# young-how/DQN-based-UAV-3D_path_planer

Hardware: NVIDIA H100
Metric: env steps/sec (+ DQN updates/sec), 500x500x100 city (higher is better)
Workload: dtype f64 env state / f32 obs+learner

## Files before the change

### dqn-based-uav-3d_path_planer_b200/csrc/tc_forward.cu

```cuda
#include "tc_forward.cuh"
#include "env_block.cuh"

#include <stdlib.h>
#include <string.h>

#include "tma.cuh"
#include "wgmma.cuh"

namespace uavrl {

static inline int rup(int x, int m) { return (x + m - 1) / m * m; }

size_t tc_smem_bytes(const TcNet &tc) { return (size_t)2 * tc.a_bytes + (size_t)tc.img_bytes + (size_t)tc.max_rows * tc.acc_ld * 4; }

int tc_build(const uavrl_learner_config &c, const NetDev &net, TcNet &tc, std::vector<int32_t> &hi_map, std::vector<int32_t> &lo_map,
             std::vector<int32_t> &hi2_map, std::vector<int32_t> &lo2_map)
{
    memset(&tc, 0, sizeof(tc));
    tc.n_layers = net.n_layers; tc.in_dim = net.in_dim; tc.n_actions = net.n_actions; tc.dueling = net.dueling;
    if (net.in_dim % 4 != 0) return -1;
    int off = 0, maxK = 0, k_pad = rup(net.in_dim, 8);
    for (int l = 0; l < net.n_layers; ++l) {
        const LayerDev &L = net.L[l];
        TcLayer &T = tc.L[l];
// ... 61 lines not shown
                if (l > 0) {
                    hi2_map[pi] = elem(T.N_pad, T.t_hi_off, k, o);
                    lo2_map[pi] = elem(T.N_pad, T.t_lo_off, k, o);
                }
            }
            hi_map[vrow ? (size_t)L.b2_off + (o - out_main) : (size_t)L.b_off + o] = tc.bias_base / 4 + T.bias_off + o;
        }
    }
    (void)c;
    return 0;
}


#define TC_TRACE(slot) do { if (a.trace && blockIdx.x == 0 && threadIdx.x == 0) a.trace[slot] = clock64(); } while (0)

template <bool FUSE_ENV, bool ACT, bool DUELING, bool FIXED>
__global__ void __launch_bounds__(kTcThreads, 1) tc_forward_kernel_t(TcNet tc, TcArgs a, EnvFuse ef)
{
    TC_TRACE(0);
    extern __shared__ __align__(1024) unsigned char smem[];
    unsigned char *Ahi = smem, *Alo = smem + tc.a_bytes, *W = smem + 2 * tc.a_bytes;
    float *acc = reinterpret_cast<float *>(W + tc.img_bytes);
    __shared__ uint64_t wbar, wbar2;
    __shared__ const float *rows[kTcTile];
    __shared__ float s_rew[kTcTile], s_done[kTcTile];

    const int tid = threadIdx.x, warp = tid >> 5, lane = tid & 31, quad = warp & 3, half = warp >> 2;
    constexpr int kCtl = kTcThreads - 32;
    const bool early_w = (a.pdl & kPdlEarlyWeights) != 0;
    const uint32_t w_split = tc.n_layers > 1 ? (uint32_t)tc.L[1].hi_off : (uint32_t)tc.img_bytes;
    auto stage_image = [&]() {
        fence_proxy_async();
// ... 71 lines not shown
            waited = true;
            if (tid == kCtl && !early_w) stage_image();
        }
        if (!wready) {
            __syncthreads();
            mbar_wait(&wbar, 0);
            wready = true;
        }
        TC_TRACE(3);
        fence_proxy_async();
        __syncthreads();
        TC_TRACE(4);

        for (int l = 0; l < tc.n_layers; ++l) {
            const TcLayer T = tc.L[l];
            mma_3xtf32<kMmaFwd, FIXED>(acc, tc.acc_ld, Ahi, Alo, W + T.hi_off, W + T.lo_off, mma_sbo(T.K_pad), T.N_pad, T.K_pad / 8, R);
            TC_TRACE(5 + 3 * l);
            if (!w2ready) { if (w_split < (uint32_t)tc.img_bytes) mbar_wait(&wbar2, 0); w2ready = true; }
            TC_TRACE(6 + 3 * l);
            const float *bias = bias_all + T.bias_off;
            const int row = quad * 32 + lane;
            const bool live = quad * 32 < R;
            if (l + 1 < tc.n_layers) {
                const uint32_t sbon = mma_sbo(T.N_pad);
                const EpiSlice e(R, kTcThreads);
                for (int c = e.c0; c < T.N_pad; c += e.step) {
                    const float4 v = e.ld(acc, tc.acc_ld, c);
                    float4 h, lo4;
                    const float x0 = fmaxf(v.x + bias[c + 0], 0.f), x1 = fmaxf(v.y + bias[c + 1], 0.f);
                    const float x2 = fmaxf(v.z + bias[c + 2], 0.f), x3 = fmaxf(v.w + bias[c + 3], 0.f);
                    tf32_split(x0, h.x, lo4.x); tf32_split(x1, h.y, lo4.y); tf32_split(x2, h.z, lo4.z); tf32_split(x3, h.w, lo4.w);
// ... 57 lines not shown
                }
                __syncthreads();
            }
        }
        if (FUSE_ENV) {
            __shared__ EnvSmem<32> env_sm;
            for (int sb = 0; sb < R; sb += 32)
                env_block<true, 32, kTcThreads, false, 8>(ef.d, env_sm, base + sb, tid, UAVRL_ACT_DISCRETE27, a.actions, ef.obs_next,
                                                       ef.reward, ef.done, nullptr, nullptr, nullptr);
            __syncthreads();
        }
    }
    TC_TRACE(20);
}

bool tc_fixed_chains(const TcNet &tc, bool train)
{
    for (int l = 0; l < tc.n_layers; ++l) {
        const TcLayer &T = tc.L[l];
        if (!mma_fixed_product(kMmaFwd, T.N_pad, T.K_pad / 8)) return false;
        if (train && l > 0 && !mma_fixed_product(kMmaDx, T.K_pad, T.N_pad / 8)) return false;
    }
    return true;
}

typedef void (*ForwardKernel)(TcNet, TcArgs, EnvFuse);
template <bool F, bool A, bool D>
static ForwardKernel pick_fwd_x(bool fixed) { return fixed ? tc_forward_kernel_t<F, A, D, true> : tc_forward_kernel_t<F, A, D, false>; }
template <bool F, bool A>
static ForwardKernel pick_fwd_d(bool dueling, bool fixed) { return dueling ? pick_fwd_x<F, A, true>(fixed) : pick_fwd_x<F, A, false>(fixed); }
static ForwardKernel pick_forward_kernel(bool fuse_env, bool act, bool dueling, bool fixed)
{
    if (fuse_env) return pick_fwd_d<true, true>(dueling, fixed);
    return act ? pick_fwd_d<false, true>(dueling, fixed) : pick_fwd_d<false, false>(dueling, fixed);
}

int launch_tc_forward(uavrl_learner *l, const TcArgs &a_in, cudaStream_t st, const EnvFuse *fuse)
{
    TcArgs a = a_in;
    const int n_sm = num_sms();
    a.rows_per_tile = (a.n >= 128 * n_sm && l->tc.max_rows == 128) ? 128 : (a.n >= 64 * n_sm) ? 64 : 32;
    a.n_tiles = (a.n + a.rows_per_tile - 1) / a.rows_per_tile;
    const int grid = a.n_tiles < n_sm ? a.n_tiles : n_sm;
    static const bool trace_on = getenv("UAVRL_TC_TRACE") != nullptr;
    long long *tr = nullptr;
    if (trace_on) { UAVRL_CUDA(cudaMalloc((void **)&tr, 32 * sizeof(long long))); UAVRL_CUDA(cudaMemset(tr, 0, 32 * sizeof(long long))); a.trace = tr; }
    const int prev = (l->pdl_chain && g_pdl.load()) ? l->pdl_prev : kPdlNone;
    a.pdl = 0;
    if (prev != kPdlNone) {
        a.pdl = kPdlOn;
        if (a.mode == kTcAct) {
            if (prev == kPdlAdam) a.pdl |= kPdlEarlyRows;
            else if (prev == kPdlEnv) a.pdl |= kPdlEarlyWeights;
        } else if (prev == kPdlEnv || prev == kPdlTd) {
            a.pdl |= kPdlEarlyWeights;
        }
    }
    EnvFuse ef;
    memset(&ef, 0, sizeof(ef));
    if (fuse) {
        ef = *fuse;
        UAVRL_CUDA(launch_kernel(pick_forward_kernel(true, a.mode == kTcAct, l->tc.dueling != 0, tc_fixed_chains(l->tc, false)), dim3(grid), dim3(kTcThreads), tc_smem_bytes(l->tc), st, a.pdl != 0, l->tc, a, ef));
        l->pdl_prev = l->pdl_chain ? kPdlEnv : kPdlNone;
    } else {
        UAVRL_CUDA(launch_kernel(pick_forward_kernel(false, a.mode == kTcAct, l->tc.dueling != 0, tc_fixed_chains(l->tc, false)), dim3(grid), dim3(kTcThreads), tc_smem_bytes(l->tc), st, a.pdl != 0, l->tc, a, ef));
        l->pdl_prev = l->pdl_chain ? (a.mode == kTcAct ? kPdlAct : kPdlTd) : kPdlNone;
    }
    UAVRL_LAUNCHED();
    if (trace_on) {
        long long h[32];
        UAVRL_CUDA(cudaStreamSynchronize(st));
        UAVRL_CUDA(cudaMemcpy(h, tr, sizeof(h), cudaMemcpyDeviceToHost));
        cudaFree(tr);
        fprintf(stderr, "[tc_trace] mode=%d n=%d R=%d grid=%d cycles since start:", a.mode, a.n, a.rows_per_tile, grid);
        for (int i = 1; i < 32; ++i) if (h[i]) fprintf(stderr, " [%d]=%lld", i, h[i] - h[0]);
        fprintf(stderr, "\n");
    }
    return 0;
}

// ... 5 lines not shown
    if (tc_smem_bytes(l->tc) > 227 * 1024) return 0;
    const size_t P = (size_t)l->net.P;
    const size_t img = (size_t)l->tc.train_img_bytes;
    UAVRL_CUDA(cudaMalloc((void **)&l->tc_img_local, img));
    UAVRL_CUDA(cudaMalloc((void **)&l->tc_img_target, img));
    UAVRL_CUDA(cudaMemset(l->tc_img_local, 0, img));
    UAVRL_CUDA(cudaMemset(l->tc_img_target, 0, img));
    int32_t **maps[] = { &l->tc_hi_map, &l->tc_lo_map, &l->tc_hi2_map, &l->tc_lo2_map };
    std::vector<int32_t> *src[] = { &hi, &lo, &hi2, &lo2 };
    for (int i = 0; i < 4; ++i) {
        UAVRL_CUDA(cudaMalloc((void **)maps[i], P * 4));
        UAVRL_CUDA(cudaMemcpy(*maps[i], src[i]->data(), P * 4, cudaMemcpyHostToDevice));
    }
    UAVRL_CUDA(cudaMalloc((void **)&l->y_buf, (size_t)l->cfg.batch_size * 4));
    UAVRL_CUDA(cudaMalloc((void **)&l->astar_buf, (size_t)l->cfg.batch_size * 4));
    const bool fixed = tc_fixed_chains(l->tc, false);
    for (int ac = 0; ac < 2; ++ac)
        for (int du = 0; du < 2; ++du)
            UAVRL_CUDA(cudaFuncSetAttribute(pick_forward_kernel(false, ac != 0, du != 0, fixed), cudaFuncAttributeMaxDynamicSharedMemorySize,
                                            (int)tc_smem_bytes(l->tc)));
    {
        l->fuse_ok = true;
        for (int du = 0; du < 2; ++du) {
            cudaFuncAttributes fa;
            UAVRL_CUDA(cudaFuncGetAttributes(&fa, pick_forward_kernel(true, true, du != 0, fixed)));
            if (fa.sharedSizeBytes + tc_smem_bytes(l->tc) > (size_t)227 * 1024) l->fuse_ok = false;
        }
        if (l->fuse_ok)
            for (int du = 0; du < 2; ++du)
                UAVRL_CUDA(cudaFuncSetAttribute(pick_forward_kernel(true, true, du != 0, fixed), cudaFuncAttributeMaxDynamicSharedMemorySize,
                                                (int)tc_smem_bytes(l->tc)));
    }
    l->y_cap = l->cfg.batch_size;
    l->tc_ok = true;
    return tc_train_init(l);
}

}
```

### dqn-based-uav-3d_path_planer_b200/csrc/tc_forward.cuh

```cuda
#pragma once
#include <vector>

#include "env.cuh"
#include "learner.cuh"

namespace uavrl {

constexpr int kTcThreads = 256;
constexpr int kTcTile = 128;

enum TcMode { kTcAct = 0, kTcArgmax = 1, kTcTdMax = 2, kTcTdGather = 3 };

struct TcArgs {
    const unsigned char *img;
    BatchSrc src;
    const float *obs;
    int32_t n, n_tiles, mode, use_next, rows_per_tile;
    float eps; int32_t is_train;
    const float *u_tape; const int32_t *rand_tape;
    uint64_t key, call;
    int32_t *actions;
    float *q_out;
    float *y_out;
    float gamma;
    int32_t pdl;
    long long *trace;
};

int tc_build(const uavrl_learner_config &c, const NetDev &net, TcNet &tc, std::vector<int32_t> &hi_map, std::vector<int32_t> &lo_map,
             std::vector<int32_t> &hi2_map, std::vector<int32_t> &lo2_map);
int tc_train_init(uavrl_learner *l);
int launch_tc_train(uavrl_learner *l, const BatchSrc &src, int B, int global_batch, const float *y, int *n_grad_parts,
                    int *n_loss_parts, cudaStream_t st, cudaEvent_t after_chain = nullptr, const AdamArgs *adam = nullptr,
                    float *loss_out = nullptr, bool *adam_done = nullptr, bool fused_td = false);
bool tc_train_can_fuse_td(const uavrl_learner *l, int B);
size_t tc_smem_bytes(const TcNet &tc);
bool tc_fixed_chains(const TcNet &tc, bool train);
struct EnvFuse { EnvDev d; float *obs_next; float *reward; uint8_t *done; };
int launch_tc_forward(uavrl_learner *l, const TcArgs &a, cudaStream_t st, const EnvFuse *fuse = nullptr);
int tc_init(uavrl_learner *l);

}
```

### dqn-based-uav-3d_path_planer_b200/csrc/tc_train.cu

```cuda
#include <string.h>
#include <stdlib.h>

#include <atomic>

#include "tc_forward.cuh"
#include "tma.cuh"
#include "wgmma.cuh"

namespace uavrl {

constexpr int kDwChunk = 128;

struct TcTrainArgs {
    const unsigned char *img;
    BatchSrc src;
    int32_t B, R, n_tiles;
    const float *y;
    float inv_global_b;
    float *act_buf, *dz_buf;
    float *loss_partials;
    int32_t loss_kind;
    int32_t fused_td, algo;
    float gamma;
    const unsigned char *img_target;
// ... 78 lines not shown
    for (int u = 0; u < 4; ++u) {
        const int i = threadIdx.x + u * kTcThreads;
        if (i < total) {
            const int r = i & (R - 1), j = i >> lgR;
            float4 h, l;
            tf32_split(v[u].x, h.x, l.x); tf32_split(v[u].y, h.y, l.y); tf32_split(v[u].z, h.z, l.z); tf32_split(v[u].w, h.w, l.w);
            const uint32_t off = mma_off(r, 4 * j, sbo);
            *reinterpret_cast<float4 *>(Ahi + off) = h;
            *reinterpret_cast<float4 *>(Alo + off) = l;
        }
    }
}

__device__ __forceinline__ uint32_t nl_split(const TcNet &tc) { return tc.n_layers > 1 ? (uint32_t)tc.L[1].hi_off : (uint32_t)tc.img_bytes; }

template <int NPRE, bool DUELING, bool FIXED>
__global__ void __launch_bounds__(kTcThreads, 1) tc_train_kernel(TcNet tc, TcTrainArgs a)
{
    TR_TRACE(0);
    extern __shared__ __align__(1024) unsigned char smem[];
    const int R = a.R;
    const uint32_t a_bytes = (uint32_t)(R / 8) * mma_sbo(tc.max_k);
    unsigned char *Ahi = smem, *Alo = smem + a_bytes, *W = smem + 2 * a_bytes;
    float *acc = reinterpret_cast<float *>(W + tc.train_img_bytes);
    __shared__ uint64_t wbar, wbar2, wbar3;
    __shared__ const float *rows[kTcTile];
    __shared__ const float *rows2[kTcTile];
    __shared__ int s_act[kTcTile], s_astar[kTcTile];
    __shared__ uint8_t s_fresh[kTcTile];
    __shared__ float s_y[kTcTile], s_rew[kTcTile], s_done[kTcTile];
    __shared__ float s_loss;

    const int tid = threadIdx.x, warp = tid >> 5, lane = tid & 31, quad = warp & 3, half = warp >> 2;
    constexpr int kCtl = kTcThreads - 32;
    if (tid == 0) s_loss = 0.f;
    constexpr bool fused = NPRE > 0;
    constexpr int n_pre = NPRE;
    uint32_t wphase = 0;
    if (tid == kCtl) {
        mbar_init(&wbar, 1); mbar_init(&wbar2, 1); mbar_init(&wbar3, 1); fence_barrier_init();
        fence_proxy_async();
        if (!fused) bulk_g2s_chunked(W, a.img, (uint32_t)tc.train_img_bytes, &wbar);
        else {
            bulk_g2s_chunked(W, (n_pre == 2) ? a.img : a.img_target, (uint32_t)tc.img_bytes, &wbar);
            if (tc.train_img_bytes > tc.img_bytes)
// ... 41 lines not shown
        for (int pass = 0; pass < n_pre; ++pass) {
            if (pass > 0 && tid == kTcThreads - 32) {
                fence_proxy_async();
                bulk_g2s_chunked(W, a.img_target, (uint32_t)tc.img_bytes, &wbar);
            }
            if (pass == 0 && early_rows) a0_store(vnext, R, tc.L[0].K_pad, Ahi, Alo);
            else build_a0(rows2, R, tc.in_dim, tc.L[0].K_pad, Ahi, Alo);
            if (pass == 0) { park_meta(); TR_TRACE(3); }
            mbar_wait(&wbar, wphase); wphase ^= 1;
            fence_proxy_async();
            __syncthreads();
            if (pass == 0) TR_TRACE(4);
            const bool td_pass = (pass == n_pre - 1);
            for (int l = 0; l < nl; ++l) {
                const TcLayer T = tc.L[l];
                mma_3xtf32<kMmaFwd, FIXED>(acc, tc.acc_ld, Ahi, Alo, W + T.hi_off, W + T.lo_off, mma_sbo(T.K_pad), T.N_pad, T.K_pad / 8, R);
                const float *bias = bias_all + T.bias_off;
                if (l + 1 < nl) {
                    const uint32_t sbon = mma_sbo(T.N_pad);
                    for (int c = e.c0; c < T.N_pad; c += e.step) {
                        const float4 v = e.ld(acc, tc.acc_ld, c);
                        float4 x, h, lo4;
                        x.x = fmaxf(v.x + bias[c + 0], 0.f); x.y = fmaxf(v.y + bias[c + 1], 0.f);
                        x.z = fmaxf(v.z + bias[c + 2], 0.f); x.w = fmaxf(v.w + bias[c + 3], 0.f);
                        tf32_split(x.x, h.x, lo4.x); tf32_split(x.y, h.y, lo4.y); tf32_split(x.z, h.z, lo4.z); tf32_split(x.w, h.w, lo4.w);
                        const uint32_t off = mma_off(e.row, c, sbon);
                        *reinterpret_cast<float4 *>(Ahi + off) = h;
                        *reinterpret_cast<float4 *>(Alo + off) = lo4;
                    }
                } else if (half == 0 && live) {
                    float q[32];
// ... 40 lines not shown
        if (!waited) { pdl_wait(); pdl_trigger(); waited = true; }
        if (n_pre == 0) park_meta();
        if (!fused && tid < R) s_y[tid] = (base + tid < a.B) ? a.y[base + tid] : 0.f;
        if (fused) { mbar_wait(&wbar, wphase); wphase ^= 1; }
        else if (!wready) { mbar_wait(&wbar, 0); wready = true; }
        fence_proxy_async();
        __syncthreads();
        TR_TRACE(10);
        const int gb = base + row;
        const bool mine = live && gb < a.B;
        const int egb = base + e.row;
        const bool emine = egb < a.B;

        for (int l = 0; l < nl; ++l) {
            const TcLayer T = tc.L[l];
            mma_3xtf32<kMmaFwd, FIXED>(acc, tc.acc_ld, Ahi, Alo, W + T.hi_off, W + T.lo_off, mma_sbo(T.K_pad), T.N_pad, T.K_pad / 8, R);
            if (fused && l == 0 && w_split < (uint32_t)tc.img_bytes) mbar_wait(&wbar2, 0);
            if (l < 4) TR_TRACE(27 + l);
            const float *bias = bias_all + T.bias_off;
            if (l + 1 < nl) {
                const uint32_t sbon = mma_sbo(T.N_pad);
                float *act_row = a.act_buf + (size_t)egb * tc.act_stride + tc.L[l + 1].act_off;
                uint32_t mk = 0u;
                for (int c = e.c0, sh = 0; c < T.N_pad; c += e.step, sh += 4) {
                    const float4 v = e.ld(acc, tc.acc_ld, c);
                    float4 x, h, lo4;
                    x.x = fmaxf(v.x + bias[c + 0], 0.f); x.y = fmaxf(v.y + bias[c + 1], 0.f);
                    x.z = fmaxf(v.z + bias[c + 2], 0.f); x.w = fmaxf(v.w + bias[c + 3], 0.f);
                    tf32_split(x.x, h.x, lo4.x); tf32_split(x.y, h.y, lo4.y); tf32_split(x.z, h.z, lo4.z); tf32_split(x.w, h.w, lo4.w);
                    const uint32_t off = mma_off(e.row, c, sbon);
                    *reinterpret_cast<float4 *>(Ahi + off) = h;
// ... 32 lines not shown
                        if (a.src.abs_err) a.src.abs_err[gb] = fabsf(diff);
                        if (a.loss_kind == 0) {
                            lterm = wb * (diff * diff);
                            gq = (2.f * diff * wb) * a.inv_global_b;
                        } else {
                            const float ad = fabsf(diff);
                            lterm = wb * (ad < 1.f ? 0.5f * (diff * diff) : ad - 0.5f);
                            gq = (fminf(fmaxf(diff, -1.f), 1.f) * wb) * a.inv_global_b;
                        }
                    }
#pragma unroll
                    for (int off = 16; off > 0; off >>= 1) lterm += __shfl_xor_sync(0xffffffffu, lterm, off);
                    TR_TRACE(23);
                    if (lane == 0) atomicAdd(&s_loss, lterm);
                    TR_TRACE(24);
                    float g[32];
                    const float inv = 1.f / (float)nA;
#pragma unroll
                    for (int j = 0; j < 32; ++j) {
                        float gj;
                        if (DUELING) gj = (j < nA) ? gq * ((j == act ? 1.f : 0.f) - inv) : (j == nA ? gq : 0.f);
                        else gj = (j == act) ? gq : 0.f;
                        g[j] = gj;
                    }
                    TR_TRACE(25);
                    float *dz_row = a.dz_buf + (size_t)gb * tc.dz_stride + T.dz_off;
#pragma unroll
                    for (int j = 0; j < 8; ++j) {
                        float4 x = make_float4(g[4 * j], g[4 * j + 1], g[4 * j + 2], g[4 * j + 3]), h, lo4;
                        tf32_split(x.x, h.x, lo4.x); tf32_split(x.y, h.y, lo4.y); tf32_split(x.z, h.z, lo4.z); tf32_split(x.w, h.w, lo4.w);
                        const uint32_t off = mma_off(row, 4 * j, sbon);
                        *reinterpret_cast<float4 *>(Ahi + off) = h;
                        *reinterpret_cast<float4 *>(Alo + off) = lo4;
                        if (mine) *reinterpret_cast<float4 *>(dz_row + 4 * j) = x;
                    }
                    TR_TRACE(26);
                }
            }
            fence_proxy_async();
            __syncthreads();
            TR_TRACE(11 + l);
        }

        if (fused && tc.train_img_bytes > tc.img_bytes) mbar_wait(&wbar3, 0);
        for (int l = nl - 1; l >= 1; --l) {
            const TcLayer T = tc.L[l];
            mma_3xtf32<kMmaDx, FIXED>(acc, tc.acc_ld, Ahi, Alo, W + T.t_hi_off, W + T.t_lo_off, mma_sbo(T.N_pad), T.K_pad, T.N_pad / 8, R);
            const uint32_t hmask = (l == 1) ? hm1 : (l == 2) ? hm2 : (l == 3) ? hm3 : hm4;
            const uint32_t sbon = mma_sbo(T.K_pad);
            float *dz_row = a.dz_buf + (size_t)egb * tc.dz_stride + tc.L[l - 1].dz_off;
            for (int c = e.c0, sh = 0; c < T.K_pad; c += e.step, sh += 4) {
                const float4 v = e.ld(acc, tc.acc_ld, c);
                const uint32_t m4 = hmask >> sh;
                float4 x, h, lo4;
                x.x = (m4 & 1u) ? v.x : 0.f; x.y = (m4 & 2u) ? v.y : 0.f;
                x.z = (m4 & 4u) ? v.z : 0.f; x.w = (m4 & 8u) ? v.w : 0.f;
                if (emine) *reinterpret_cast<float4 *>(dz_row + c) = x;
                if (l > 1) {
                    tf32_split(x.x, h.x, lo4.x); tf32_split(x.y, h.y, lo4.y); tf32_split(x.z, h.z, lo4.z); tf32_split(x.w, h.w, lo4.w);
                    const uint32_t off = mma_off(e.row, c, sbon);
                    *reinterpret_cast<float4 *>(Ahi + off) = h;
                    *reinterpret_cast<float4 *>(Alo + off) = lo4;
                }
            }
            fence_proxy_async();
            __syncthreads();
            TR_TRACE(16 + l);
        }
    }
    TR_TRACE(20);
    if (tid == 0) a.loss_partials[blockIdx.x] = s_loss;
}

constexpr uint32_t kDwSbo = (kDwChunk / 4) * 128u + 16u;
constexpr int kDwARows = 128;

template <int LOG2F4, int U>
__device__ __forceinline__ void dw_load_rows(const float *const *rows, int width, float4 (&v)[U])
{
#pragma unroll
    for (int u = 0; u < U; ++u) {
        const int i = threadIdx.x + u * kTcThreads;
        const int b = i >> LOG2F4, jc = i & ((1 << LOG2F4) - 1);
        const float *r = (b < kDwChunk) ? rows[b] : nullptr;
        v[u] = (r && 4 * jc < width) ? __ldg(reinterpret_cast<const float4 *>(r) + jc) : make_float4(0.f, 0.f, 0.f, 0.f);
    }
// ... 197 lines not shown
        const float g = (g4[0] + g4[1]) + (g4[2] + g4[3]);
        a.ptrs.grad[i] = g;
        adam_update_one(a.adam, a.ptrs, i, g);
    }
    if (blockIdx.x == 0 && warp == 7 && a.ptrs.loss_out) {
        float sl = 0.f;
        for (int c = lane; c < a.adam.n_loss_parts; c += 32) sl += __ldcg(a.ptrs.loss_partials + c);
#pragma unroll
        for (int off = 16; off > 0; off >>= 1) sl += __shfl_xor_sync(0xffffffffu, sl, off);
        if (lane == 0) *a.ptrs.loss_out = sl * a.adam.inv_b;
    }
}

typedef void (*TrainKernel)(TcNet, TcTrainArgs);
template <int N, bool D>
static TrainKernel pick_train_x(bool fixed) { return fixed ? tc_train_kernel<N, D, true> : tc_train_kernel<N, D, false>; }
template <int N>
static TrainKernel pick_train_d(bool dueling, bool fixed) { return dueling ? pick_train_x<N, true>(fixed) : pick_train_x<N, false>(fixed); }
static TrainKernel pick_train_kernel(int npre, bool dueling, bool fixed)
{
    return npre == 0 ? pick_train_d<0>(dueling, fixed) : npre == 1 ? pick_train_d<1>(dueling, fixed) : pick_train_d<2>(dueling, fixed);
}

static size_t train_smem_bytes(const TcNet &tc, int R)
{
    return (size_t)2 * (R / 8) * mma_sbo(tc.max_k) + (size_t)tc.train_img_bytes + (size_t)R * tc.acc_ld * 4;
}
static size_t dw_smem_bytes(const TcNet &tc)
{
    int maxN = 32;
    for (int l = 0; l < tc.n_layers; ++l) if (tc.L[l].N_pad > maxN) maxN = tc.L[l].N_pad;
    return (size_t)2 * ((kDwARows + maxN) / 8) * kDwSbo;
}

int tc_train_init(uavrl_learner *l)
{
    l->tc_train_ok = false;
    const TcNet &tc = l->tc;
    for (int i = 0; i < tc.n_layers; ++i)
        if (tc.L[i].K_real + 1 > 128 || tc.L[i].K_real % 4 != 0 || (tc.L[i].N_pad != 32 && tc.L[i].N_pad != 64)) return 0;
    if (train_smem_bytes(tc, 32) > 227 * 1024 || dw_smem_bytes(tc) > 227 * 1024) return 0;
    if (train_smem_bytes(tc, 32) < (size_t)(32 / 8) * mma_sbo(tc.max_k) + (size_t)8 * mma_sbo(tc.max_k)) return 0;
    for (int np = 0; np < 3; ++np)
        for (int du = 0; du < 2; ++du)
            UAVRL_CUDA(cudaFuncSetAttribute(pick_train_kernel(np, du != 0, tc_fixed_chains(tc, true)), cudaFuncAttributeMaxDynamicSharedMemorySize,
                                            (int)(train_smem_bytes(tc, 64) <= 227 * 1024 ? train_smem_bytes(tc, 64) : train_smem_bytes(tc, 32))));
    UAVRL_CUDA(cudaFuncSetAttribute(tc_dw_kernel<false>, cudaFuncAttributeMaxDynamicSharedMemorySize, (int)dw_smem_bytes(tc)));
    UAVRL_CUDA(cudaFuncSetAttribute(tc_dw_kernel<true>, cudaFuncAttributeMaxDynamicSharedMemorySize, (int)dw_smem_bytes(tc)));
    const size_t cap = (size_t)l->cfg.batch_size;
    UAVRL_CUDA(cudaMalloc((void **)&l->act_buf, cap * (size_t)(tc.act_stride > 0 ? tc.act_stride : 4) * 4));
    UAVRL_CUDA(cudaMalloc((void **)&l->dz_buf, cap * (size_t)tc.dz_stride * 4));
    l->train_cap = (int32_t)cap;
    l->tc_train_ok = true;
    return 0;
}

std::atomic<int> g_fuse_td{1};
static int train_rows_per_tile(const TcNet &tc, int B)
{
    return (B > 32 * num_sms() && train_smem_bytes(tc, 64) <= 227 * 1024) ? 64 : 32;
}
// ... 14 lines not shown
    memset(&a, 0, sizeof(a));
    a.img = l->tc_img_local; a.src = src; a.B = B; a.y = y; a.inv_global_b = 1.0f / (float)global_batch;
    a.act_buf = l->act_buf; a.dz_buf = l->dz_buf; a.loss_partials = l->loss_partials;
    a.loss_kind = l->cfg.loss_kind;
    a.fused_td = fused_td ? 1 : 0; a.algo = l->cfg.algo; a.gamma = l->cfg.gamma; a.img_target = l->tc_img_target;
    a.R = train_rows_per_tile(tc, B);
    a.n_tiles = (B + a.R - 1) / a.R;
    const int grid = a.n_tiles < num_sms() ? a.n_tiles : num_sms();
    const bool chain = l->pdl_chain && g_pdl.load();
    if (fused_td && a.n_tiles > grid) return fail(UAVRL_ERR_INVALID, "fused TD needs one tile per CTA");
    static const bool trace_on = getenv("UAVRL_TC_TRACE") != nullptr;
    long long *tr = nullptr;
    if (trace_on) { UAVRL_CUDA(cudaMalloc((void **)&tr, 48 * sizeof(long long))); UAVRL_CUDA(cudaMemset(tr, 0, 48 * sizeof(long long))); a.trace = tr + 16; }
    const bool use_pdl = chain && (fused_td ? (l->pdl_prev == kPdlEnv) : (l->pdl_prev == kPdlTd));
    const int npre = fused_td ? (l->cfg.algo != UAVRL_ALGO_DQN ? 2 : 1) : 0;
    auto train_fn = pick_train_kernel(npre, tc.dueling != 0, tc_fixed_chains(tc, true));
    UAVRL_CUDA(launch_kernel(train_fn, dim3(grid), dim3(kTcThreads), train_smem_bytes(tc, a.R), st, use_pdl, tc, a));
    static const bool twice = trace_on && getenv("UAVRL_TRAIN_TWICE") != nullptr;
    if (twice) UAVRL_CUDA(launch_kernel(train_fn, dim3(grid), dim3(kTcThreads), train_smem_bytes(tc, a.R), st, false, tc, a));
    l->pdl_prev = chain ? kPdlTrain : kPdlNone;
    UAVRL_LAUNCHED();
    if (after_chain) UAVRL_CUDA(cudaEventRecord(after_chain, st));
    TcDwArgs d;
    memset(&d, 0, sizeof(d));
    d.src = src; d.B = B; d.n_chunks = (B + kDwChunk - 1) / kDwChunk; d.P = l->net.P;
    d.act_buf = l->act_buf; d.dz_buf = l->dz_buf; d.partials = l->partials;
    const int n_sm = num_sms();
    const int max_slices = n_sm / tc.n_layers > 0 ? n_sm / tc.n_layers : 1;
    d.n_slices = d.n_chunks < max_slices ? d.n_chunks : max_slices;
    const int dw_grid = d.n_slices * tc.n_layers;
    const bool fuse = adam != nullptr && g_fuse_dw_adam.load() && dw_grid <= n_sm;
// ... 46 lines not shown
```

### dqn-based-uav-3d_path_planer_b200/csrc/wgmma.cuh

```cuda
#pragma once
#include <stdint.h>

namespace uavrl {

constexpr uint32_t kMmaLBO = 128;

__host__ __device__ constexpr uint32_t mma_sbo(int k_pad) { return (uint32_t)(k_pad / 4) * 128u; }
__host__ __device__ constexpr uint32_t mma_tile_bytes(int rows, int k_pad) { return (uint32_t)(rows / 8) * mma_sbo(k_pad); }

__device__ __forceinline__ uint32_t mma_off(int r, int c, uint32_t sbo, uint32_t lbo = kMmaLBO)
{
    return (uint32_t)(r >> 3) * sbo + (uint32_t)(c >> 2) * lbo + (uint32_t)(r & 7) * 16u + (uint32_t)(c & 3) * 4u;
}

__device__ __forceinline__ uint64_t mma_desc(const void *smem_ptr, uint32_t sbo, uint32_t lbo = kMmaLBO)
{
    const uint32_t addr = (uint32_t)__cvta_generic_to_shared(smem_ptr);
    uint64_t d = 0;
    d |= (uint64_t)((addr >> 4) & 0x3FFFu);
    d |= (uint64_t)((lbo >> 4) & 0x3FFFu) << 16;
    d |= (uint64_t)((sbo >> 4) & 0x3FFFu) << 32;
    return d;
}

// ... 39 lines not shown
template <int N>
__device__ __forceinline__ void wgmma_3xtf32(float *d, uint64_t a_hi, uint64_t a_lo, uint64_t b_hi, uint64_t b_lo, int ksteps,
                                             uint32_t accumulate)
{
    const uint64_t kStep = (uint64_t)((2 * kMmaLBO) >> 4);
    fence_operands<N>(d);
    wgmma_fence();
    for (int k = 0; k < ksteps; ++k) wgmma_tf32<N>(d, a_hi + k * kStep, b_hi + k * kStep, (k > 0 || accumulate) ? 1u : 0u);
    for (int k = 0; k < ksteps; ++k) wgmma_tf32<N>(d, a_hi + k * kStep, b_lo + k * kStep, 1u);
    for (int k = 0; k < ksteps; ++k) wgmma_tf32<N>(d, a_lo + k * kStep, b_hi + k * kStep, 1u);
    wgmma_commit();
    wgmma_wait0();
    fence_operands<N>(d);
}

template <int N, int KS>
__device__ __forceinline__ void wgmma_3xtf32_k(float *d, uint64_t a_hi, uint64_t a_lo, uint64_t b_hi, uint64_t b_lo)
{
    const uint64_t kStep = (uint64_t)((2 * kMmaLBO) >> 4);
    fence_operands<N>(d);
    wgmma_fence();
#pragma unroll
    for (int k = 0; k < KS; ++k) wgmma_tf32<N>(d, a_hi + k * kStep, b_hi + k * kStep, k > 0 ? 1u : 0u);
#pragma unroll
    for (int k = 0; k < KS; ++k) wgmma_tf32<N>(d, a_hi + k * kStep, b_lo + k * kStep, 1u);
#pragma unroll
    for (int k = 0; k < KS; ++k) wgmma_tf32<N>(d, a_lo + k * kStep, b_hi + k * kStep, 1u);
    wgmma_commit();
    wgmma_wait0();
    fence_operands<N>(d);
}

enum MmaKind { kMmaFwd = 0, kMmaDx = 1 };

__host__ __device__ constexpr bool mma_fixed(int kind, int n, int ksteps)
{
    return kind == kMmaFwd ? (n == 64 && (ksteps == 13 || ksteps == 8 || ksteps == 16)) || (n == 32 && ksteps == 8)
                           : n == 64 && (ksteps == 4 || ksteps == 8);
}
__host__ __device__ constexpr bool mma_fixed_product(int kind, int n, int ksteps)
{
    return (n < 64 || mma_fixed(kind, 64, ksteps)) && (n % 64 < 32 || mma_fixed(kind, 32, ksteps)) && n % 32 == 0;
}

template <int N, int KIND>
__device__ __forceinline__ void wgmma_3xtf32_fixed(float *d, uint64_t a_hi, uint64_t a_lo, uint64_t b_hi, uint64_t b_lo, int ksteps)
{
    if constexpr (mma_fixed(KIND, N, 4)) if (ksteps == 4) wgmma_3xtf32_k<N, 4>(d, a_hi, a_lo, b_hi, b_lo);
    if constexpr (mma_fixed(KIND, N, 8)) if (ksteps == 8) wgmma_3xtf32_k<N, 8>(d, a_hi, a_lo, b_hi, b_lo);
    if constexpr (mma_fixed(KIND, N, 13)) if (ksteps == 13) wgmma_3xtf32_k<N, 13>(d, a_hi, a_lo, b_hi, b_lo);
    if constexpr (mma_fixed(KIND, N, 16)) if (ksteps == 16) wgmma_3xtf32_k<N, 16>(d, a_hi, a_lo, b_hi, b_lo);
}

template <int N>
__device__ __forceinline__ void store_frag(const float *d, float *acc, int ld, int row0, int col0, int R)
{
    const int t = threadIdx.x & 127, r = row0 + 16 * (t >> 5) + ((t & 31) >> 2), c = col0 + 2 * (t & 3);
#pragma unroll
    for (int i = 0; i < N / 8; ++i) {
        if (r < R) *reinterpret_cast<float2 *>(acc + (size_t)r * ld + c + 8 * i) = make_float2(d[4 * i], d[4 * i + 1]);
        if (r + 8 < R) *reinterpret_cast<float2 *>(acc + (size_t)(r + 8) * ld + c + 8 * i) = make_float2(d[4 * i + 2], d[4 * i + 3]);
    }
}

template <int N, int KIND, bool FIXED>
__device__ __forceinline__ void mma_chunk(float *acc, int ld, int row0, int n0, uint64_t a_hi, uint64_t a_lo, const unsigned char *b_hi,
                                          const unsigned char *b_lo, uint32_t sbo, int ksteps, int R)
{
    float d[N / 2];
    const uint32_t boff = (uint32_t)(n0 >> 3) * sbo;
    const uint64_t bh = mma_desc(b_hi + boff, sbo), bl = mma_desc(b_lo + boff, sbo);
    if (FIXED) wgmma_3xtf32_fixed<N, KIND>(d, a_hi, a_lo, bh, bl, ksteps);
    else wgmma_3xtf32<N>(d, a_hi, a_lo, bh, bl, ksteps, 0u);
    store_frag<N>(d, acc, ld, row0, n0, R);
}

template <int KIND, bool FIXED>
__device__ __forceinline__ void mma_3xtf32(float *acc, int ld, const unsigned char *a_hi, const unsigned char *a_lo,
                                           const unsigned char *b_hi, const unsigned char *b_lo, uint32_t sbo, int N, int ksteps, int R)
{
    const int row0 = (threadIdx.x >> 7) * 64;
    if (row0 < R) {
        const uint64_t ah = mma_desc(a_hi + (row0 >> 3) * sbo, sbo), al = mma_desc(a_lo + (row0 >> 3) * sbo, sbo);
        int n0 = 0;
        for (; n0 + 64 <= N; n0 += 64) mma_chunk<64, KIND, FIXED>(acc, ld, row0, n0, ah, al, b_hi, b_lo, sbo, ksteps, R);
        if (n0 + 32 <= N) { mma_chunk<32, KIND, FIXED>(acc, ld, row0, n0, ah, al, b_hi, b_lo, sbo, ksteps, R); n0 += 32; }
        if (!FIXED && n0 < N) mma_chunk<16, KIND, FIXED>(acc, ld, row0, n0, ah, al, b_hi, b_lo, sbo, ksteps, R);
    }
    __syncthreads();
}

__device__ __forceinline__ void acc_ld32(const float *acc, int ld, int row, int c0, float (&v)[32])
{
    const float4 *src = reinterpret_cast<const float4 *>(acc + (size_t)row * ld + c0);
#pragma unroll
    for (int j = 0; j < 8; ++j) {
        const float4 t = src[j];
// ... 19 lines not shown
```

Measured before the change: 74.47 million.

## Add transposed wgmma path for 32-row tiles to use both warpgroups

For 32-row tiles, adds a transposed 3xTF32 wgmma variant that computes W·Xᵀ, so the layer's output features fill the M=64 dimension and the batch rows become N=32. The work is split across both warpgroups by feature block, and results are written back transposed into the accumulator. Before, the second warpgroup sat idle and half of each M=64 instruction was wasted on padding rows. The train kernel's output-gradient epilogue is also spread across all threads through a shared gq array instead of one thread per row. This adds template instantiations and kernel variants, strided scalar shared-memory stores with possible bank conflicts, and an extra barrier.

```diff
diff --git a/dqn-based-uav-3d_path_planer_b200/csrc/tc_forward.cu b/dqn-based-uav-3d_path_planer_b200/csrc/tc_forward.cu
--- a/dqn-based-uav-3d_path_planer_b200/csrc/tc_forward.cu
+++ b/dqn-based-uav-3d_path_planer_b200/csrc/tc_forward.cu
@@ -99,8 +99,8 @@
 
 #define TC_TRACE(slot) do { if (a.trace && blockIdx.x == 0 && threadIdx.x == 0) a.trace[slot] = clock64(); } while (0)
 
-template <bool FUSE_ENV, bool ACT, bool DUELING, bool FIXED>
-__global__ void __launch_bounds__(kTcThreads, 1) tc_forward_kernel_t(TcNet tc, TcArgs a, EnvFuse ef)
+template <bool FUSE_ENV, bool ACT, bool DUELING, bool FIXED, bool T32>
+__device__ __forceinline__ void tc_forward_body(const TcNet &tc, const TcArgs &a, const EnvFuse &ef)
 {
     TC_TRACE(0);
     extern __shared__ __align__(1024) unsigned char smem[];
@@ -202,7 +202,7 @@
 
         for (int l = 0; l < tc.n_layers; ++l) {
             const TcLayer T = tc.L[l];
-            mma_3xtf32<kMmaFwd, FIXED>(acc, tc.acc_ld, Ahi, Alo, W + T.hi_off, W + T.lo_off, mma_sbo(T.K_pad), T.N_pad, T.K_pad / 8, R);
+            mma_3xtf32<kMmaFwd, FIXED, T32>(acc, tc.acc_ld, Ahi, Alo, W + T.hi_off, W + T.lo_off, mma_sbo(T.K_pad), T.N_pad, T.K_pad / 8, R);
             TC_TRACE(5 + 3 * l);
             if (!w2ready) { if (w_split < (uint32_t)tc.img_bytes) mbar_wait(&wbar2, 0); w2ready = true; }
             TC_TRACE(6 + 3 * l);
@@ -290,6 +290,17 @@
     TC_TRACE(20);
 }
 
+template <bool FUSE_ENV, bool ACT, bool DUELING, bool FIXED>
+__global__ void __launch_bounds__(kTcThreads, 1) tc_forward_kernel_t(TcNet tc, TcArgs a, EnvFuse ef)
+{
+    tc_forward_body<FUSE_ENV, ACT, DUELING, FIXED, false>(tc, a, ef);
+}
+template <bool FUSE_ENV, bool ACT, bool DUELING>
+__global__ void __launch_bounds__(kTcThreads, 1) tc_forward_kernel_t32(TcNet tc, TcArgs a, EnvFuse ef)
+{
+    tc_forward_body<FUSE_ENV, ACT, DUELING, true, true>(tc, a, ef);
+}
+
 bool tc_fixed_chains(const TcNet &tc, bool train)
 {
     for (int l = 0; l < tc.n_layers; ++l) {
@@ -300,16 +311,31 @@
     return true;
 }
 
+bool tc_t32_chains(const TcNet &tc, bool train)
+{
+    if (!tc_fixed_chains(tc, train)) return false;
+    for (int l = 0; l < tc.n_layers; ++l) {
+        const TcLayer &T = tc.L[l];
+        if (T.N_pad >= 64 && !mma_fixed_t(kMmaFwd, T.K_pad / 8)) return false;
+        if (train && l > 0 && !mma_fixed_t(kMmaDx, T.N_pad / 8)) return false;
+    }
+    return true;
+}
+
 typedef void (*ForwardKernel)(TcNet, TcArgs, EnvFuse);
 template <bool F, bool A, bool D>
-static ForwardKernel pick_fwd_x(bool fixed) { return fixed ? tc_forward_kernel_t<F, A, D, true> : tc_forward_kernel_t<F, A, D, false>; }
+static ForwardKernel pick_fwd_x(int chains)
+{
+    return chains == 2 ? tc_forward_kernel_t32<F, A, D> : chains == 1 ? tc_forward_kernel_t<F, A, D, true> : tc_forward_kernel_t<F, A, D, false>;
+}
 template <bool F, bool A>
-static ForwardKernel pick_fwd_d(bool dueling, bool fixed) { return dueling ? pick_fwd_x<F, A, true>(fixed) : pick_fwd_x<F, A, false>(fixed); }
-static ForwardKernel pick_forward_kernel(bool fuse_env, bool act, bool dueling, bool fixed)
-{
-    if (fuse_env) return pick_fwd_d<true, true>(dueling, fixed);
-    return act ? pick_fwd_d<false, true>(dueling, fixed) : pick_fwd_d<false, false>(dueling, fixed);
-}
+static ForwardKernel pick_fwd_d(bool dueling, int chains) { return dueling ? pick_fwd_x<F, A, true>(chains) : pick_fwd_x<F, A, false>(chains); }
+static ForwardKernel pick_forward_kernel(bool fuse_env, bool act, bool dueling, int chains)
+{
+    if (fuse_env) return pick_fwd_d<true, true>(dueling, chains);
+    return act ? pick_fwd_d<false, true>(dueling, chains) : pick_fwd_d<false, false>(dueling, chains);
+}
+static int fwd_chains(const TcNet &tc, int R) { return (R == 32 && tc_t32_chains(tc, false)) ? 2 : tc_fixed_chains(tc, false) ? 1 : 0; }
 
 int launch_tc_forward(uavrl_learner *l, const TcArgs &a_in, cudaStream_t st, const EnvFuse *fuse)
 {
@@ -336,10 +362,10 @@
     memset(&ef, 0, sizeof(ef));
     if (fuse) {
         ef = *fuse;
-        UAVRL_CUDA(launch_kernel(pick_forward_kernel(true, a.mode == kTcAct, l->tc.dueling != 0, tc_fixed_chains(l->tc, false)), dim3(grid), dim3(kTcThreads), tc_smem_bytes(l->tc), st, a.pdl != 0, l->tc, a, ef));
+        UAVRL_CUDA(launch_kernel(pick_forward_kernel(true, a.mode == kTcAct, l->tc.dueling != 0, fwd_chains(l->tc, a.rows_per_tile)), dim3(grid), dim3(kTcThreads), tc_smem_bytes(l->tc), st, a.pdl != 0, l->tc, a, ef));
         l->pdl_prev = l->pdl_chain ? kPdlEnv : kPdlNone;
     } else {
-        UAVRL_CUDA(launch_kernel(pick_forward_kernel(false, a.mode == kTcAct, l->tc.dueling != 0, tc_fixed_chains(l->tc, false)), dim3(grid), dim3(kTcThreads), tc_smem_bytes(l->tc), st, a.pdl != 0, l->tc, a, ef));
+        UAVRL_CUDA(launch_kernel(pick_forward_kernel(false, a.mode == kTcAct, l->tc.dueling != 0, fwd_chains(l->tc, a.rows_per_tile)), dim3(grid), dim3(kTcThreads), tc_smem_bytes(l->tc), st, a.pdl != 0, l->tc, a, ef));
         l->pdl_prev = l->pdl_chain ? (a.mode == kTcAct ? kPdlAct : kPdlTd) : kPdlNone;
     }
     UAVRL_LAUNCHED();
@@ -375,22 +401,25 @@
     }
     UAVRL_CUDA(cudaMalloc((void **)&l->y_buf, (size_t)l->cfg.batch_size * 4));
     UAVRL_CUDA(cudaMalloc((void **)&l->astar_buf, (size_t)l->cfg.batch_size * 4));
-    const bool fixed = tc_fixed_chains(l->tc, false);
-    for (int ac = 0; ac < 2; ++ac)
-        for (int du = 0; du < 2; ++du)
-            UAVRL_CUDA(cudaFuncSetAttribute(pick_forward_kernel(false, ac != 0, du != 0, fixed), cudaFuncAttributeMaxDynamicSharedMemorySize,
-                                            (int)tc_smem_bytes(l->tc)));
+    const int chains[2] = {fwd_chains(l->tc, 32), fwd_chains(l->tc, 64)};
+    for (int ch = 0; ch < 2; ++ch)
+        for (int ac = 0; ac < 2; ++ac)
+            for (int du = 0; du < 2; ++du)
+                UAVRL_CUDA(cudaFuncSetAttribute(pick_forward_kernel(false, ac != 0, du != 0, chains[ch]), cudaFuncAttributeMaxDynamicSharedMemorySize,
+                                                (int)tc_smem_bytes(l->tc)));
     {
         l->fuse_ok = true;
-        for (int du = 0; du < 2; ++du) {
-            cudaFuncAttributes fa;
-            UAVRL_CUDA(cudaFuncGetAttributes(&fa, pick_forward_kernel(true, true, du != 0, fixed)));
-            if (fa.sharedSizeBytes + tc_smem_bytes(l->tc) > (size_t)227 * 1024) l->fuse_ok = false;
-        }
+        for (int ch = 0; ch < 2; ++ch)
+            for (int du = 0; du < 2; ++du) {
+                cudaFuncAttributes fa;
+                UAVRL_CUDA(cudaFuncGetAttributes(&fa, pick_forward_kernel(true, true, du != 0, chains[ch])));
+                if (fa.sharedSizeBytes + tc_smem_bytes(l->tc) > (size_t)227 * 1024) l->fuse_ok = false;
+            }
         if (l->fuse_ok)
-            for (int du = 0; du < 2; ++du)
-                UAVRL_CUDA(cudaFuncSetAttribute(pick_forward_kernel(true, true, du != 0, fixed), cudaFuncAttributeMaxDynamicSharedMemorySize,
-                                                (int)tc_smem_bytes(l->tc)));
+            for (int ch = 0; ch < 2; ++ch)
+                for (int du = 0; du < 2; ++du)
+                    UAVRL_CUDA(cudaFuncSetAttribute(pick_forward_kernel(true, true, du != 0, chains[ch]), cudaFuncAttributeMaxDynamicSharedMemorySize,
+                                                    (int)tc_smem_bytes(l->tc)));
     }
     l->y_cap = l->cfg.batch_size;
     l->tc_ok = true;
diff --git a/dqn-based-uav-3d_path_planer_b200/csrc/tc_forward.cuh b/dqn-based-uav-3d_path_planer_b200/csrc/tc_forward.cuh
--- a/dqn-based-uav-3d_path_planer_b200/csrc/tc_forward.cuh
+++ b/dqn-based-uav-3d_path_planer_b200/csrc/tc_forward.cuh
@@ -36,6 +36,7 @@
 bool tc_train_can_fuse_td(const uavrl_learner *l, int B);
 size_t tc_smem_bytes(const TcNet &tc);
 bool tc_fixed_chains(const TcNet &tc, bool train);
+bool tc_t32_chains(const TcNet &tc, bool train);
 struct EnvFuse { EnvDev d; float *obs_next; float *reward; uint8_t *done; };
 int launch_tc_forward(uavrl_learner *l, const TcArgs &a, cudaStream_t st, const EnvFuse *fuse = nullptr);
 int tc_init(uavrl_learner *l);
diff --git a/dqn-based-uav-3d_path_planer_b200/csrc/tc_train.cu b/dqn-based-uav-3d_path_planer_b200/csrc/tc_train.cu
--- a/dqn-based-uav-3d_path_planer_b200/csrc/tc_train.cu
+++ b/dqn-based-uav-3d_path_planer_b200/csrc/tc_train.cu
@@ -116,8 +116,8 @@
 
 __device__ __forceinline__ uint32_t nl_split(const TcNet &tc) { return tc.n_layers > 1 ? (uint32_t)tc.L[1].hi_off : (uint32_t)tc.img_bytes; }
 
-template <int NPRE, bool DUELING, bool FIXED>
-__global__ void __launch_bounds__(kTcThreads, 1) tc_train_kernel(TcNet tc, TcTrainArgs a)
+template <int NPRE, bool DUELING, bool FIXED, bool T32>
+__device__ __forceinline__ void tc_train_body(const TcNet &tc, const TcTrainArgs &a)
 {
     TR_TRACE(0);
     extern __shared__ __align__(1024) unsigned char smem[];
@@ -131,6 +131,7 @@
     __shared__ int s_act[kTcTile], s_astar[kTcTile];
     __shared__ uint8_t s_fresh[kTcTile];
     __shared__ float s_y[kTcTile], s_rew[kTcTile], s_done[kTcTile];
+    __shared__ float s_gq[kTcTile];
     __shared__ float s_loss;
 
     const int tid = threadIdx.x, warp = tid >> 5, lane = tid & 31, quad = warp & 3, half = warp >> 2;
@@ -202,7 +203,7 @@
             const bool td_pass = (pass == n_pre - 1);
             for (int l = 0; l < nl; ++l) {
                 const TcLayer T = tc.L[l];
-                mma_3xtf32<kMmaFwd, FIXED>(acc, tc.acc_ld, Ahi, Alo, W + T.hi_off, W + T.lo_off, mma_sbo(T.K_pad), T.N_pad, T.K_pad / 8, R);
+                mma_3xtf32<kMmaFwd, FIXED, T32>(acc, tc.acc_ld, Ahi, Alo, W + T.hi_off, W + T.lo_off, mma_sbo(T.K_pad), T.N_pad, T.K_pad / 8, R);
                 const float *bias = bias_all + T.bias_off;
                 if (l + 1 < nl) {
                     const uint32_t sbon = mma_sbo(T.N_pad);
@@ -273,7 +274,7 @@
 
         for (int l = 0; l < nl; ++l) {
             const TcLayer T = tc.L[l];
-            mma_3xtf32<kMmaFwd, FIXED>(acc, tc.acc_ld, Ahi, Alo, W + T.hi_off, W + T.lo_off, mma_sbo(T.K_pad), T.N_pad, T.K_pad / 8, R);
+            mma_3xtf32<kMmaFwd, FIXED, T32>(acc, tc.acc_ld, Ahi, Alo, W + T.hi_off, W + T.lo_off, mma_sbo(T.K_pad), T.N_pad, T.K_pad / 8, R);
             if (fused && l == 0 && w_split < (uint32_t)tc.img_bytes) mbar_wait(&wbar2, 0);
             if (l < 4) TR_TRACE(27 + l);
             const float *bias = bias_all + T.bias_off;
@@ -336,28 +337,29 @@
                     TR_TRACE(23);
                     if (lane == 0) atomicAdd(&s_loss, lterm);
                     TR_TRACE(24);
-                    float g[32];
-                    const float inv = 1.f / (float)nA;
-#pragma unroll
-                    for (int j = 0; j < 32; ++j) {
-                        float gj;
-                        if (DUELING) gj = (j < nA) ? gq * ((j == act ? 1.f : 0.f) - inv) : (j == nA ? gq : 0.f);
-                        else gj = (j == act) ? gq : 0.f;
-                        g[j] = gj;
+                    s_gq[row] = gq;
+                }
+                __syncthreads();
+                TR_TRACE(25);
+                const int nA = tc.n_actions, act = s_act[e.row];
+                const float gq = s_gq[e.row], inv = 1.f / (float)nA;
+                float *dz_row = a.dz_buf + (size_t)egb * tc.dz_stride + T.dz_off;
+                for (int c = e.c0; c < T.N_pad; c += e.step) {
+                    float g[4];
+#pragma unroll
+                    for (int jj = 0; jj < 4; ++jj) {
+                        const int j = c + jj;
+                        if (DUELING) g[jj] = (j < nA) ? gq * ((j == act ? 1.f : 0.f) - inv) : (j == nA ? gq : 0.f);
+                        else g[jj] = (j == act) ? gq : 0.f;
                     }
-                    TR_TRACE(25);
-                    float *dz_row = a.dz_buf + (size_t)gb * tc.dz_stride + T.dz_off;
-#pragma unroll
-                    for (int j = 0; j < 8; ++j) {
-                        float4 x = make_float4(g[4 * j], g[4 * j + 1], g[4 * j + 2], g[4 * j + 3]), h, lo4;
-                        tf32_split(x.x, h.x, lo4.x); tf32_split(x.y, h.y, lo4.y); tf32_split(x.z, h.z, lo4.z); tf32_split(x.w, h.w, lo4.w);
-                        const uint32_t off = mma_off(row, 4 * j, sbon);
-                        *reinterpret_cast<float4 *>(Ahi + off) = h;
-                        *reinterpret_cast<float4 *>(Alo + off) = lo4;
-                        if (mine) *reinterpret_cast<float4 *>(dz_row + 4 * j) = x;
-                    }
-                    TR_TRACE(26);
+                    float4 x = make_float4(g[0], g[1], g[2], g[3]), h, lo4;
+                    tf32_split(x.x, h.x, lo4.x); tf32_split(x.y, h.y, lo4.y); tf32_split(x.z, h.z, lo4.z); tf32_split(x.w, h.w, lo4.w);
+                    const uint32_t off = mma_off(e.row, c, sbon);
+                    *reinterpret_cast<float4 *>(Ahi + off) = h;
+                    *reinterpret_cast<float4 *>(Alo + off) = lo4;
+                    if (emine) *reinterpret_cast<float4 *>(dz_row + c) = x;
                 }
+                TR_TRACE(26);
             }
             fence_proxy_async();
             __syncthreads();
@@ -367,7 +369,7 @@
         if (fused && tc.train_img_bytes > tc.img_bytes) mbar_wait(&wbar3, 0);
         for (int l = nl - 1; l >= 1; --l) {
             const TcLayer T = tc.L[l];
-            mma_3xtf32<kMmaDx, FIXED>(acc, tc.acc_ld, Ahi, Alo, W + T.t_hi_off, W + T.t_lo_off, mma_sbo(T.N_pad), T.K_pad, T.N_pad / 8, R);
+            mma_3xtf32<kMmaDx, FIXED, T32>(acc, tc.acc_ld, Ahi, Alo, W + T.t_hi_off, W + T.t_lo_off, mma_sbo(T.N_pad), T.K_pad, T.N_pad / 8, R);
             const uint32_t hmask = (l == 1) ? hm1 : (l == 2) ? hm2 : (l == 3) ? hm3 : hm4;
             const uint32_t sbon = mma_sbo(T.K_pad);
             float *dz_row = a.dz_buf + (size_t)egb * tc.dz_stride + tc.L[l - 1].dz_off;
@@ -392,6 +394,17 @@
     }
     TR_TRACE(20);
     if (tid == 0) a.loss_partials[blockIdx.x] = s_loss;
+}
+
+template <int NPRE, bool DUELING, bool FIXED>
+__global__ void __launch_bounds__(kTcThreads, 1) tc_train_kernel(TcNet tc, TcTrainArgs a)
+{
+    tc_train_body<NPRE, DUELING, FIXED, false>(tc, a);
+}
+template <int NPRE, bool DUELING>
+__global__ void __launch_bounds__(kTcThreads, 1) tc_train_kernel_t32(TcNet tc, TcTrainArgs a)
+{
+    tc_train_body<NPRE, DUELING, true, true>(tc, a);
 }
 
 constexpr uint32_t kDwSbo = (kDwChunk / 4) * 128u + 16u;
@@ -619,13 +632,17 @@
 
 typedef void (*TrainKernel)(TcNet, TcTrainArgs);
 template <int N, bool D>
-static TrainKernel pick_train_x(bool fixed) { return fixed ? tc_train_kernel<N, D, true> : tc_train_kernel<N, D, false>; }
+static TrainKernel pick_train_x(int chains)
+{
+    return chains == 2 ? tc_train_kernel_t32<N, D> : chains == 1 ? tc_train_kernel<N, D, true> : tc_train_kernel<N, D, false>;
+}
 template <int N>
-static TrainKernel pick_train_d(bool dueling, bool fixed) { return dueling ? pick_train_x<N, true>(fixed) : pick_train_x<N, false>(fixed); }
-static TrainKernel pick_train_kernel(int npre, bool dueling, bool fixed)
-{
-    return npre == 0 ? pick_train_d<0>(dueling, fixed) : npre == 1 ? pick_train_d<1>(dueling, fixed) : pick_train_d<2>(dueling, fixed);
-}
+static TrainKernel pick_train_d(bool dueling, int chains) { return dueling ? pick_train_x<N, true>(chains) : pick_train_x<N, false>(chains); }
+static TrainKernel pick_train_kernel(int npre, bool dueling, int chains)
+{
+    return npre == 0 ? pick_train_d<0>(dueling, chains) : npre == 1 ? pick_train_d<1>(dueling, chains) : pick_train_d<2>(dueling, chains);
+}
+static int train_chains(const TcNet &tc, int R) { return (R == 32 && tc_t32_chains(tc, true)) ? 2 : tc_fixed_chains(tc, true) ? 1 : 0; }
 
 static size_t train_smem_bytes(const TcNet &tc, int R)
 {
@@ -646,10 +663,11 @@
         if (tc.L[i].K_real + 1 > 128 || tc.L[i].K_real % 4 != 0 || (tc.L[i].N_pad != 32 && tc.L[i].N_pad != 64)) return 0;
     if (train_smem_bytes(tc, 32) > 227 * 1024 || dw_smem_bytes(tc) > 227 * 1024) return 0;
     if (train_smem_bytes(tc, 32) < (size_t)(32 / 8) * mma_sbo(tc.max_k) + (size_t)8 * mma_sbo(tc.max_k)) return 0;
-    for (int np = 0; np < 3; ++np)
-        for (int du = 0; du < 2; ++du)
-            UAVRL_CUDA(cudaFuncSetAttribute(pick_train_kernel(np, du != 0, tc_fixed_chains(tc, true)), cudaFuncAttributeMaxDynamicSharedMemorySize,
-                                            (int)(train_smem_bytes(tc, 64) <= 227 * 1024 ? train_smem_bytes(tc, 64) : train_smem_bytes(tc, 32))));
+    for (int R = 32; R <= 64; R += 32)
+        for (int np = 0; np < 3; ++np)
+            for (int du = 0; du < 2; ++du)
+                UAVRL_CUDA(cudaFuncSetAttribute(pick_train_kernel(np, du != 0, train_chains(tc, R)), cudaFuncAttributeMaxDynamicSharedMemorySize,
+                                                (int)(train_smem_bytes(tc, 64) <= 227 * 1024 ? train_smem_bytes(tc, 64) : train_smem_bytes(tc, 32))));
     UAVRL_CUDA(cudaFuncSetAttribute(tc_dw_kernel<false>, cudaFuncAttributeMaxDynamicSharedMemorySize, (int)dw_smem_bytes(tc)));
     UAVRL_CUDA(cudaFuncSetAttribute(tc_dw_kernel<true>, cudaFuncAttributeMaxDynamicSharedMemorySize, (int)dw_smem_bytes(tc)));
     const size_t cap = (size_t)l->cfg.batch_size;
@@ -694,7 +712,7 @@
     if (trace_on) { UAVRL_CUDA(cudaMalloc((void **)&tr, 48 * sizeof(long long))); UAVRL_CUDA(cudaMemset(tr, 0, 48 * sizeof(long long))); a.trace = tr + 16; }
     const bool use_pdl = chain && (fused_td ? (l->pdl_prev == kPdlEnv) : (l->pdl_prev == kPdlTd));
     const int npre = fused_td ? (l->cfg.algo != UAVRL_ALGO_DQN ? 2 : 1) : 0;
-    auto train_fn = pick_train_kernel(npre, tc.dueling != 0, tc_fixed_chains(tc, true));
+    auto train_fn = pick_train_kernel(npre, tc.dueling != 0, train_chains(tc, a.R));
     UAVRL_CUDA(launch_kernel(train_fn, dim3(grid), dim3(kTcThreads), train_smem_bytes(tc, a.R), st, use_pdl, tc, a));
     static const bool twice = trace_on && getenv("UAVRL_TRAIN_TWICE") != nullptr;
     if (twice) UAVRL_CUDA(launch_kernel(train_fn, dim3(grid), dim3(kTcThreads), train_smem_bytes(tc, a.R), st, false, tc, a));
diff --git a/dqn-based-uav-3d_path_planer_b200/csrc/wgmma.cuh b/dqn-based-uav-3d_path_planer_b200/csrc/wgmma.cuh
--- a/dqn-based-uav-3d_path_planer_b200/csrc/wgmma.cuh
+++ b/dqn-based-uav-3d_path_planer_b200/csrc/wgmma.cuh
@@ -77,7 +77,7 @@
     fence_operands<N>(d);
 }
 
-template <int N, int KS>
+template <int N, int KS, bool T = false>
 __device__ __forceinline__ void wgmma_3xtf32_k(float *d, uint64_t a_hi, uint64_t a_lo, uint64_t b_hi, uint64_t b_lo)
 {
     const uint64_t kStep = (uint64_t)((2 * kMmaLBO) >> 4);
@@ -86,9 +86,9 @@
 #pragma unroll
     for (int k = 0; k < KS; ++k) wgmma_tf32<N>(d, a_hi + k * kStep, b_hi + k * kStep, k > 0 ? 1u : 0u);
 #pragma unroll
-    for (int k = 0; k < KS; ++k) wgmma_tf32<N>(d, a_hi + k * kStep, b_lo + k * kStep, 1u);
-#pragma unroll
-    for (int k = 0; k < KS; ++k) wgmma_tf32<N>(d, a_lo + k * kStep, b_hi + k * kStep, 1u);
+    for (int k = 0; k < KS; ++k) wgmma_tf32<N>(d, (T ? a_lo : a_hi) + k * kStep, (T ? b_hi : b_lo) + k * kStep, 1u);
+#pragma unroll
+    for (int k = 0; k < KS; ++k) wgmma_tf32<N>(d, (T ? a_hi : a_lo) + k * kStep, (T ? b_lo : b_hi) + k * kStep, 1u);
     wgmma_commit();
     wgmma_wait0();
     fence_operands<N>(d);
@@ -106,13 +106,17 @@
     return (n < 64 || mma_fixed(kind, 64, ksteps)) && (n % 64 < 32 || mma_fixed(kind, 32, ksteps)) && n % 32 == 0;
 }
 
-template <int N, int KIND>
+__host__ __device__ constexpr bool mma_fixed_t(int kind, int ksteps)
+{
+    return kind == kMmaFwd ? (ksteps == 13 || ksteps == 8) : (ksteps == 4 || ksteps == 8);
+}
+template <int N, int KIND, bool T = false>
 __device__ __forceinline__ void wgmma_3xtf32_fixed(float *d, uint64_t a_hi, uint64_t a_lo, uint64_t b_hi, uint64_t b_lo, int ksteps)
 {
-    if constexpr (mma_fixed(KIND, N, 4)) if (ksteps == 4) wgmma_3xtf32_k<N, 4>(d, a_hi, a_lo, b_hi, b_lo);
-    if constexpr (mma_fixed(KIND, N, 8)) if (ksteps == 8) wgmma_3xtf32_k<N, 8>(d, a_hi, a_lo, b_hi, b_lo);
-    if constexpr (mma_fixed(KIND, N, 13)) if (ksteps == 13) wgmma_3xtf32_k<N, 13>(d, a_hi, a_lo, b_hi, b_lo);
-    if constexpr (mma_fixed(KIND, N, 16)) if (ksteps == 16) wgmma_3xtf32_k<N, 16>(d, a_hi, a_lo, b_hi, b_lo);
+    if constexpr (T ? mma_fixed_t(KIND, 4) : mma_fixed(KIND, N, 4)) if (ksteps == 4) wgmma_3xtf32_k<N, 4, T>(d, a_hi, a_lo, b_hi, b_lo);
+    if constexpr (T ? mma_fixed_t(KIND, 8) : mma_fixed(KIND, N, 8)) if (ksteps == 8) wgmma_3xtf32_k<N, 8, T>(d, a_hi, a_lo, b_hi, b_lo);
+    if constexpr (T ? mma_fixed_t(KIND, 13) : mma_fixed(KIND, N, 13)) if (ksteps == 13) wgmma_3xtf32_k<N, 13, T>(d, a_hi, a_lo, b_hi, b_lo);
+    if constexpr (T ? mma_fixed_t(KIND, 16) : mma_fixed(KIND, N, 16)) if (ksteps == 16) wgmma_3xtf32_k<N, 16, T>(d, a_hi, a_lo, b_hi, b_lo);
 }
 
 template <int N>
@@ -123,6 +127,16 @@
     for (int i = 0; i < N / 8; ++i) {
         if (r < R) *reinterpret_cast<float2 *>(acc + (size_t)r * ld + c + 8 * i) = make_float2(d[4 * i], d[4 * i + 1]);
         if (r + 8 < R) *reinterpret_cast<float2 *>(acc + (size_t)(r + 8) * ld + c + 8 * i) = make_float2(d[4 * i + 2], d[4 * i + 3]);
+    }
+}
+
+__device__ __forceinline__ void store_frag_t32(const float *d, float *acc, int ld, int col0)
+{
+    const int t = threadIdx.x & 127, f = col0 + 16 * (t >> 5) + ((t & 31) >> 2), s = 2 * (t & 3);
+#pragma unroll
+    for (int i = 0; i < 4; ++i) {
+        float *p = acc + (size_t)(s + 8 * i) * ld + f;
+        p[0] = d[4 * i]; p[ld] = d[4 * i + 1]; p[8] = d[4 * i + 2]; p[ld + 8] = d[4 * i + 3];
     }
 }
 
@@ -138,12 +152,22 @@
     store_frag<N>(d, acc, ld, row0, n0, R);
 }
 
-template <int KIND, bool FIXED>
+template <int KIND, bool FIXED, bool T32 = false>
 __device__ __forceinline__ void mma_3xtf32(float *acc, int ld, const unsigned char *a_hi, const unsigned char *a_lo,
                                            const unsigned char *b_hi, const unsigned char *b_lo, uint32_t sbo, int N, int ksteps, int R)
 {
+    static_assert(FIXED || !T32, "the transposed chains exist as compile-time chains only");
     const int row0 = (threadIdx.x >> 7) * 64;
-    if (row0 < R) {
+    if constexpr (T32) {
+        const uint64_t xh = mma_desc(a_hi, sbo), xl = mma_desc(a_lo, sbo);
+        for (int f0 = row0; f0 + 64 <= N; f0 += 128) {
+            float d[16];
+            const uint32_t woff = (uint32_t)(f0 >> 3) * sbo;
+            wgmma_3xtf32_fixed<32, KIND, true>(d, mma_desc(b_hi + woff, sbo), mma_desc(b_lo + woff, sbo), xh, xl, ksteps);
+            store_frag_t32(d, acc, ld, f0);
+        }
+        if (N % 64 == 32 && row0 == 0) mma_chunk<32, KIND, true>(acc, ld, 0, N - 32, xh, xl, b_hi, b_lo, sbo, ksteps, R);
+    } else if (row0 < R) {
         const uint64_t ah = mma_desc(a_hi + (row0 >> 3) * sbo, sbo), al = mma_desc(a_lo + (row0 >> 3) * sbo, sbo);
         int n0 = 0;
         for (; n0 + 64 <= N; n0 += 64) mma_chunk<64, KIND, FIXED>(acc, ld, row0, n0, ah, al, b_hi, b_lo, sbo, ksteps, R);
```

Measured after the change: 77.01 million (median of 6 runs). +3.4%, better.
